# OpenRobotLab/EmbodiedScan

Measured on AMD Instinct MI355X. Metric: scans/sec (train step) mv-3ddet, 20x(480x640) RGB-D views, higher is better.
Workload: dtype bf16; 1 GPU; mv-3ddet ResNet-50(w16) + MinkResNet34 + FCAF3DHeadRotMat, 20 views 480x640, 100k points/scan, bf16 matrix cores with f32 accumulate / f32 master weights, full train step incl. H2D of the batch and AdamW; views=20, parallelism=dp1, h2d=157 MB per step as ONE copy from a pinned slab on a copy stream, double-buffered

## Files before the change

### embodiedscan_amd/csrc/rowops.hip

```cpp
#include "common.h"
#include "../../include/es_hip.h"

int ES_OPT_NORM_CHUNK = 0;
static int norm_chunk_rows(int max_rows) {
  if (ES_OPT_NORM_CHUNK > 0) return ES_OPT_NORM_CHUNK;
  return max_rows <= (1 << 17) ? 128 : (max_rows <= (1 << 18) ? 256 : 512);
}
#define FCH 16
#define FST 64

struct Segs { int n; int off[ES_MAX_SEG + 1]; };
__device__ inline int seg_of(const Segs& s, int row) {
  int g = 0;
  for (int i = 1; i < s.n; ++i) g += (row >= s.off[i]);
  return g;
}
static Segs make_segs(const int* seg_off, int nseg) {
  Segs s;
  s.n = nseg;
  for (int i = 0; i <= nseg; ++i) s.off[i] = seg_off[i];
  return s;
}
static int max_seg_rows(const Segs& s) {
  int m = 0;
// ... 258 lines not shown
                    (((((uintptr_t)x) | ((uintptr_t)y) | ((uintptr_t)res) | ((uintptr_t)weight) | ((uintptr_t)bias) |
                       ((uintptr_t)mean) | ((uintptr_t)invstd)) & 15) == 0);
  if (vec0 && norm_cb_ok(n, C, nseg) && seg_off[0] == 0 && seg_off[1] == n) {
    hipLaunchKernelGGL(k_norm_fwd_cb, dim3(C / 16), dim3(4 * NCB_TY), 0, st, x, ldx, n, C, eps, weight, bias, res, ldr, act,
                       running_mean, running_var, momentum, mean, invstd, y, ldy, (unsigned short*)y_bf16);
    ES_CHECK_LAUNCH();
    return 0;
  }
  const int NCH = norm_chunk_rows(max_seg_rows(s));
  int nchunk = es_cdiv(max_seg_rows(s), NCH);
  if (nchunk < 1) nchunk = 1;
  hipLaunchKernelGGL(k_norm_stats, dim3(nchunk, nseg), dim3(256), 0, st, x, ldx, C, s, nchunk, NCH,
                     workspace);
  hipLaunchKernelGGL(k_norm_finalize, dim3(es_cdiv(C, FCH), nseg), dim3(FCH * FST), 0, st, workspace, C, s, nchunk, NCH, eps,
                     mean, invstd, running_mean, running_var, momentum);
  const bool vec = ((C & 3) == 0) && ((ldx & 3) == 0) && ((ldy & 3) == 0) && (!res || (ldr & 3) == 0) &&
                   (((((uintptr_t)x) | ((uintptr_t)y) | ((uintptr_t)res) | ((uintptr_t)weight) | ((uintptr_t)bias) |
                      ((uintptr_t)mean) | ((uintptr_t)invstd)) & 15) == 0);
  if (vec) {
    int g = es_cdiv((long long)n * (C >> 2), 512);
    if (g > 8192) g = 8192;
    hipLaunchKernelGGL(k_norm_apply4, dim3(g < 1 ? 1 : g), dim3(256), 0, st, x, ldx, n, C, s, mean, invstd, weight, bias,
                       res, ldr, act, y, ldy, (unsigned short*)y_bf16);
  } else {
    int g = es_cdiv((long long)n * C, 256);
    if (g > 4096) g = 4096;
    hipLaunchKernelGGL(k_norm_apply, dim3(g), dim3(256), 0, st, x, ldx, n, C, s, mean, invstd, weight, bias, res,
                       ldr, act, y, ldy);
    if (y_bf16) return es_cast_rows_bf16(y, ldy, n, C, y_bf16, stream);
  }
  ES_CHECK_LAUNCH();
  return 0;
}
extern "C" size_t es_norm_workspace_floats(int n, int C, const int* seg_off, int nseg) {
  int m = 0;
  for (int i = 0; i < nseg; ++i) m = max(m, seg_off[i + 1] - seg_off[i]);
  int nchunk = es_cdiv(m, norm_chunk_rows(m));
  if (nchunk < 1) nchunk = 1;
  return (size_t)nseg * nchunk * 2 * C;
}

__global__ __launch_bounds__(256) void k_norm_bwd_stats(float* __restrict__ dy, int ldd, const float* __restrict__ y,
                                                        int ldy, const float* __restrict__ x, int ldx, int C, Segs segs,
                                                        int nchunk, int NCH, const float* __restrict__ mean,
                                                        const float* __restrict__ invstd, int act,
                                                        float* __restrict__ partial) {
  __shared__ float4 red[2][256];
  int seg = blockIdx.y, chunk = blockIdx.x;
  int r0 = segs.off[seg] + chunk * NCH, r1 = min(segs.off[seg + 1], r0 + NCH);
  float* out = partial + ((size_t)(seg * nchunk + chunk) * 2) * C;
  const bool vec = ((C & 3) == 0) && ((ldx & 3) == 0) && ((ldd & 3) == 0) && ((ldy & 3) == 0) &&
                   ((((uintptr_t)x) & 15) == 0) && ((((uintptr_t)dy) & 15) == 0) && ((((uintptr_t)y) & 15) == 0);
  if (!vec) {
    for (int c = threadIdx.x; c < C; c += blockDim.x) {
      float s = 0.f, q = 0.f, m = mean[seg * C + c], is = invstd[seg * C + c];
      for (int r = r0; r < r1; ++r) {
        float g = dy[(size_t)r * ldd + c];
        if (act) {
          float yv = y[(size_t)r * ldy + c];
          g = (act == 1) ? (yv > 0.f ? g : 0.f) : (yv > 0.f ? g : g * (yv + 1.f));
          dy[(size_t)r * ldd + c] = g;
        }
        s += g;
        q += g * ((x[(size_t)r * ldx + c] - m) * is);
      }
      out[c] = s;
      out[C + c] = q;
    }
    return;
  }
// ... 239 lines not shown
    const bool vec0 = ((C & 3) == 0) && ((ldx & 3) == 0) && ((ldd & 3) == 0) && ((ldo & 3) == 0) && ((ldy & 3) == 0) &&
                      (((((uintptr_t)x) | ((uintptr_t)dy) | ((uintptr_t)dx) | ((uintptr_t)y) | ((uintptr_t)weight) |
                         ((uintptr_t)mean) | ((uintptr_t)invstd)) & 15) == 0);
    if (vec0 && dx != dy && ES_OPT_NORM_CB_BWD && norm_cb_ok(n, C, nseg) && seg_off[0] == 0 && seg_off[1] == n) {
      hipLaunchKernelGGL(k_norm_bwd_cb, dim3(C / 16), dim3(4 * NCB_TY), 0, st, dy, ldd, y, ldy, x, ldx, n, C, mean, invstd, weight, act,
                         dweight, dbias, dx, ldo, accumulate, (unsigned short*)dx_bf16);
      ES_CHECK_LAUNCH();
      return 0;
    }
  }
  float* sums = workspace + (size_t)nseg * nchunk * 2 * C;
  hipLaunchKernelGGL(k_norm_bwd_stats, dim3(nchunk, nseg), dim3(256), 0, st, dy, ldd, y, ldy, x,
                     ldx, C, s, nchunk, NCH, mean, invstd, act, workspace);
  hipLaunchKernelGGL(k_norm_bwd_finalize, dim3(es_cdiv(C, FCH)), dim3(FCH * FST), 0, st, workspace, C, s, nchunk, NCH, sums,
                     sums + (size_t)nseg * C, dweight, dbias);
  const bool vec = ((C & 3) == 0) && ((ldx & 3) == 0) && ((ldd & 3) == 0) && ((ldo & 3) == 0) &&
                   (((((uintptr_t)x) | ((uintptr_t)dy) | ((uintptr_t)dx) | ((uintptr_t)weight) | ((uintptr_t)mean) |
                      ((uintptr_t)invstd) | ((uintptr_t)sums)) & 15) == 0) && ((((size_t)nseg * C) & 3) == 0);
  if (vec && dx != dy) {
    int g = es_cdiv((long long)n * (C >> 2), 512);
    if (g > 8192) g = 8192;
    hipLaunchKernelGGL(k_norm_bwd_apply4, dim3(g < 1 ? 1 : g), dim3(256), 0, st, dy, ldd, x, ldx, n, C, s, mean, invstd,
                       weight, sums, sums + (size_t)nseg * C, dx, ldo, accumulate, (unsigned short*)dx_bf16);
  } else {
    int g = es_cdiv((long long)n * C, 256);
    if (g > 4096) g = 4096;
    hipLaunchKernelGGL(k_norm_bwd_apply, dim3(g), dim3(256), 0, st, dy, ldd, x, ldx, n, C, s, mean, invstd, weight,
                       sums, sums + (size_t)nseg * C, dx, ldo, accumulate);
    if (dx_bf16) return es_cast_rows_bf16(dx, ldo, n, C, dx_bf16, stream);
  }
  ES_CHECK_LAUNCH();
  return 0;
}

__global__ void k_maxpool_fwd(const float* __restrict__ x, int ldx, const int* __restrict__ nbr, int n_out, int K,
                              int C, float* __restrict__ y, int* __restrict__ arg) {
  size_t tot = (size_t)n_out * C;
  for (size_t e = (size_t)blockIdx.x * blockDim.x + threadIdx.x; e < tot; e += (size_t)gridDim.x * blockDim.x) {
    int j = (int)(e / C), c = (int)(e - (size_t)j * C);
    float best = -INFINITY;
    int bi = -1;
    for (int k = 0; k < K; ++k) {
      int i = nbr[(size_t)j * K + k];
      if (i < 0) continue;
      float v = x[(size_t)i * ldx + c];
      if (bi < 0 || v > best) { best = v; bi = i; }
    }
    y[e] = best;
    arg[e] = bi;
  }
}
extern "C" int es_maxpool_fwd(const float* x, int ldx, const int* nbr, int n_out, int K, int C, float* y, int* arg,
                              void* stream) {
  if (n_out <= 0) return 0;
  int g = es_cdiv((long long)n_out * C, 256);
  if (g > 4096) g = 4096;
  hipLaunchKernelGGL(k_maxpool_fwd, dim3(g), dim3(256), 0, (hipStream_t)stream, x, ldx, nbr, n_out, K, C, y, arg);
  ES_CHECK_LAUNCH();
  return 0;
}
__global__ void k_maxpool_fwd_h(const float* __restrict__ x, int ldx, const int* __restrict__ nbr, int n_out, int K, int C,
                                unsigned short* __restrict__ y) {
  size_t tot = (size_t)n_out * C;
  for (size_t e = (size_t)blockIdx.x * blockDim.x + threadIdx.x; e < tot; e += (size_t)gridDim.x * blockDim.x) {
    int j = (int)(e / C), c = (int)(e - (size_t)j * C);
    float best = -INFINITY;
// ... 552 lines not shown
```

### embodiedscan_amd/csrc/spconv.hip

```cpp
#include "common.h"
#include "../../include/es_hip.h"

typedef float f32x4 __attribute__((ext_vector_type(4)));

static int ES_OPT_PINGPONG = 1;
static int ES_OPT_WGRAD_HUGE = 1;
static int ES_OPT_ROWGEMM = 1;
static int ES_OPT_WG_BIG_TARGET = 2048;
static int ES_OPT_WG_BIG_ROWS = 512;
static int ES_OPT_WG_SMALL_TARGET = 1024;
static int ES_OPT_WG_CAP_MB = 256;
static int ES_OPT_FWD_SPLIT_WGS = 384;
static int ES_OPT_DMA = 2;
static int ES_OPT_DMA_MIN_CIN = 768;
static int ES_OPT_WGRAD_TR = 1;
static int ES_OPT_ROWGEMM2 = 1;
static int ES_OPT_SPLIT_FOLD = 0;
static int ES_OPT_RG128_MIN_CIN = 0;
static int ES_OPT_NARROW_SLICES = 768;
static int ES_OPT_LIN_SMALL = 256;
static int ES_OPT_EXPAND = 65536;
static int ES_OPT_EXPAND_WGS = 1024;
static int ES_OPT_RG320 = 1;
static int ES_OPT_NARROW = 1;
static int ES_OPT_WSHARE = 0;
static int ES_OPT_RG128_MIN_WGS = 0;
extern int ES_OPT_NORM_CB_ROWS;
extern int ES_OPT_NORM_CB_BWD;
extern int ES_OPT_ELECT_SAFE;
extern int ES_OPT_NORM_CHUNK;
extern "C" int es_set_option(int key, int value) {
  if (key == 1) { ES_OPT_PINGPONG = value; return 0; }
  if (key == 2) { ES_OPT_WGRAD_HUGE = value; return 0; }
  if (key == 3) { ES_OPT_ROWGEMM = value; return 0; }
  if (key == 4) { ES_OPT_WG_BIG_TARGET = value; return 0; }
  if (key == 5) { ES_OPT_WG_BIG_ROWS = value; return 0; }
  if (key == 6) { ES_OPT_WG_SMALL_TARGET = value; return 0; }
  if (key == 7) { ES_OPT_WG_CAP_MB = value; return 0; }
  if (key == 8) { ES_OPT_FWD_SPLIT_WGS = value; return 0; }
  if (key == 9) { ES_OPT_NORM_CHUNK = value; return 0; }
  if (key == 10) { ES_OPT_DMA = value; return 0; }
  if (key == 11) { ES_OPT_DMA_MIN_CIN = value; return 0; }
  if (key == 12) { ES_OPT_RG128_MIN_CIN = value; return 0; }
  if (key == 13) { ES_OPT_ROWGEMM2 = value; return 0; }
  if (key == 14) { ES_OPT_WGRAD_TR = value; return 0; }
  if (key == 15) { ES_OPT_NORM_CB_ROWS = value; return 0; }
  if (key == 16) { ES_OPT_SPLIT_FOLD = value; return 0; }
  if (key == 17) { ES_OPT_NORM_CB_BWD = value; return 0; }
  if (key == 18) { ES_OPT_ELECT_SAFE = value; return 0; }
  if (key == 19) { ES_OPT_RG128_MIN_WGS = value; return 0; }
  if (key == 20) { ES_OPT_WSHARE = value; return 0; }
  if (key == 21) { ES_OPT_NARROW = value; return 0; }
  if (key == 22) { ES_OPT_NARROW_SLICES = value; return 0; }
  if (key == 23) { ES_OPT_RG320 = value; return 0; }
  if (key == 24) { ES_OPT_LIN_SMALL = value; return 0; }
  if (key == 25) { ES_OPT_EXPAND = value; return 0; }
  if (key == 26) { ES_OPT_EXPAND_WGS = value; return 0; }
  return -2;
}


#define BM 128
#define BN 64
#define BK 16
#define LDB (BN + 16)
#define MAXK 27

__device__ inline int a_swz(int row_k) { return (((row_k >> 2) & 3) << 3) ^ ((row_k & 1) << 4); }

template <bool TRANS_W>
__global__ __launch_bounds__(256) void k_spconv(const float* __restrict__ X, int ldx, const float* __restrict__ W,
                                                const int* __restrict__ nbr, int n_out, int n_in, int K, int Cin,
                                                int Cout, const float* __restrict__ bias, float* __restrict__ Y,
                                                int ldy, int accumulate) {
  __shared__ float As[BK * BM];
  __shared__ float Bs[BK * LDB];
  __shared__ int nbrS[BM * MAXK];
  __shared__ int tapAny[32];

  const int t = threadIdx.x, lane = t & 63, wv = t >> 6;
  const int row0 = blockIdx.x * BM, n0 = blockIdx.y * BN;
  const bool vecA = ((ldx & 3) == 0) && ((((uintptr_t)X) & 15) == 0);
  const bool vecB = TRANS_W ? (((Cin & 3) == 0) && ((((uintptr_t)W) & 15) == 0))
                            : (((Cout & 3) == 0) && ((((uintptr_t)W) & 15) == 0));

  if (t < 32) tapAny[t] = 0;
  __syncthreads();
  for (int e = t; e < BM * K; e += 256) {
    int r = e / K, k = e - r * K;
    int j = row0 + r, v = -1;
// ... 2674 lines not shown
```

### embodiedscan_amd/engine.py

```python
import os

import torch
from . import hip
from .hip import P, call, iarr


def _stream():
    return hip.stream()


_NEW_VARS = None


class Var:
    __slots__ = ('d', 'g', 'rg', 'dh', 'gh', 'gate', 'gated', 'fresh')

    def __init__(self, d, rg=True):
        self.d, self.g, self.rg = d, None, rg
        self.dh = self.gh = None
        if _NEW_VARS is not None:
            _NEW_VARS.append(self)
        self.fresh = False
        self.gate = None
        self.gated = False
# ... 407 lines not shown
def _cast_rows(t):
    n, C = t.shape
    h = torch.empty((n, C), dtype=torch.bfloat16, device=t.device)
    call('es_cast_rows_bf16', P(t), t.stride(0), n, C, P(h), _stream())
    return h


GEN_FUSED = [os.environ.get('ES_GEN_FUSED', '1') != '0']


def _split_ws(n_out, K, cin, cout, like):
    if K <= 1 or n_out <= 0:
        return None, 0
    nf = int(hip.raw('es_spconv_split_workspace_floats')(n_out, K, cin, cout))
    if nf == 0:
        return None, 0
    return ticket_ws(nf, like, tag='split')


def _fwd_bf16(X, x_is_bf16, ldx, Wp, nbr, n_out, n_in, K, cin, cout, bias_p, Y, ldy, acc, like):
    ws, nf = _split_ws(n_out, K, cin, cout, like)
    if ws is not None:
        call('es_spconv_fwd_bf16_ws', X, x_is_bf16, ldx, Wp, nbr, n_out, n_in, K, cin, cout, bias_p, Y, ldy, acc, P(ws), nf, _stream())
        return 'es_spconv_fwd_bf16_ws'
    call('es_spconv_fwd_bf16', X, x_is_bf16, ldx, Wp, nbr, n_out, n_in, K, cin, cout, bias_p, Y, ldy, acc, _stream())
    return 'es_spconv_fwd_bf16'


def _use_shadow(n_rows, C, K, cin, cout):
    return K > 1 and hip.raw('es_spconv_bf16_is_fast')(n_rows, C, K, cin, cout) == 1


HALO = [os.environ.get('ES_HALO', '1') != '0']
if os.environ.get('ES_HALO_MIN_WGS') is not None:
    hip.raw('es_halo_set_option')(30, int(os.environ['ES_HALO_MIN_WGS']))


def _halo_ok(nbr, n_out, n_in, ldx, K, cin, cout):
    return (HALO[0] and K == 27 and nbr is not None
            and hip.raw('es_spconv_halo_supported')(n_out, n_in, ldx, K, cin, cout) == 1)


def halo_plan(nbr):
    plan = getattr(nbr, '_halo', None)
    if plan is None:
        n_out, K = nbr.shape
        rows = int(hip.raw('es_halo_plan_rows')(n_out))
        loc = torch.empty((rows, K), dtype=torch.int16, device=nbr.device)
        hrows = torch.empty((rows // 256, 256 * K), dtype=torch.int32, device=nbr.device)
        hcnt = torch.empty((rows // 256,), dtype=torch.int32, device=nbr.device)
        call('es_halo_plan', P(nbr), n_out, K, P(loc), P(hrows), P(hcnt), _stream())
        plan = nbr._halo = (loc, hrows, hcnt)
        if hip.PROFILE is not None:
            hip.PAIRS[loc.data_ptr()] = (nbr >= 0).sum()
    return plan


def _halo_launch(Xh, ldx, Wp, nbr, n_out, n_in, K, cin, cout, bias_p, Y, ldy, acc):
    fwd = getattr(nbr, '_mirror_of', None)
    loc, hrows, hcnt = halo_plan(fwd if fwd is not None else nbr)
    return hip.try_call('es_spconv_halo_bf16', Xh, ldx, Wp, P(loc), P(hrows), P(hcnt), n_out, n_in, K, cin, cout, bias_p, Y, ldy, acc,
                        int(fwd is not None), _stream())


def empty(shape, like, dtype=torch.float32):
    return torch.empty(shape, dtype=dtype, device=like.device)
# ... 347 lines not shown
            x.shadow()
            sw = _wgrad_stream(y.g, x.d, gh, x.dh)
            _required(_dense_wgrad(P(x.dh), cin, P(gh), cout, dense, 1, cin, cout, P(w.g), _first_write(P(w.g)), sw, gh))
        if x.rg:
            g, acc = _grad_target(x, x.d)
            _required(_dense_launch(P(gh), cout, P(w.bf16()[0]), dense, 4, cin, cout, P(g), _ld(g), acc, gh))
        if DEBUG_CONV is not None:
            B, X, Y, Z = dense[:4]
            gv = y.g.view(B, X, 2, Y, 2, Z, 2, cout)
            recs = [dict(x=x.d, w=ParamSlice(w, k), nbr=None, n_out=n, gy=gv[:, :, k >> 2, :, (k >> 1) & 1, :, k & 1].reshape(n, cout).clone(),
                         bf=True, gate=None, need_dx=bool(x.rg), before=rec_before, bias=None, bias_from=0, group=id(y), group_size=8)
                    for k in range(8)]
            if x.rg:
                recs[-1]['after'] = x.g.clone()
            DEBUG_CONV.extend(recs)
    TAPE.add(bwd)
    return y


def norm(x, weight, bias, seg_off, eps, act=0, res=None, running=None, momentum=0.1):
    n, C = x.d.shape
    nseg = len(seg_off) - 1
    so = iarr(seg_off)
    ws_n = hip.raw('es_norm_workspace_floats')(n, C, so, nseg) + 2 * nseg * C
    ws = empty((ws_n,), x.d)
    mean, invstd = empty((nseg, C), x.d), empty((nseg, C), x.d)
    y = Var(empty((n, C), x.d))
    rm, rv = (running if running is not None else (None, None))
    fuse = PRECISION[0] == 'bf16' and C >= 16 and C % 8 == 0
    private, x.fresh = bool(x.fresh), False
    if fuse:
        y.dh = empty((n, C), x.d, dtype=torch.bfloat16)
    run0 = (rm.clone(), rv.clone()) if (DEBUG_FWD is not None and rm is not None) else (None, None)
    call('es_norm_fwd', P(x.d), _ld(x.d), n, C, so, nseg, float(eps), P(weight.d), P(bias.d),
         P(res.d) if res is not None else 0, _ld(res.d) if res is not None else 0, act, P(rm), P(rv), float(momentum),
         P(mean), P(invstd), P(ws), P(y.d), C, P(y.dh) if fuse else 0, _stream())
    if DEBUG_FWD is not None:
        fwd_record('norm', 'es_norm_fwd', x=x.d, w=weight.d, b=bias.d, seg_off=list(seg_off), eps=float(eps), act=act,
                   res=res.d if res is not None else None, rm0=run0[0], rv0=run0[1], rm1=rm, rv1=rv, momentum=float(momentum),
                   mean=mean, invstd=invstd, y=y.d, yh=y.dh if fuse else None)

    def bwd():
        if y.g is None:
            return
        s = _stream()
        if DEBUG_GRADS is not None:
            DEBUG_GRADS[id(y)] = y.g.clone()
        ws2 = empty((ws_n,), x.d)
        g, acc = _grad_target(x, x.d)
        gh = empty((n, C), x.d, dtype=torch.bfloat16) if (fuse and private and _ld(g) == C) else None
        call('es_norm_bwd', P(y.g), _ld(y.g), P(y.d), C, P(x.d), _ld(x.d), n, C, so, nseg, P(mean), P(invstd),
             P(weight.d), act, P(weight.g), P(bias.g), P(ws2), P(g), _ld(g), acc, P(gh), s)
        x.gh = gh
        if DEBUG_GRADS is not None:
            DEBUG_GRADS[('norm', id(y))] = dict(dx=g.clone(), dz=y.g.clone(), mean=mean.clone(), invstd=invstd.clone(),
                                                x=x.d.clone(), yd=y.d.clone(), acc=acc, n=n, C=C, act=act)
        if res is not None and res.rg:
            if res.g is None:
                res.g = y.g
            else:
                call('es_axpy2d', P(res.g), _ld(res.g), P(y.g), _ld(y.g), n, C, 1.0, 1, s)
    TAPE.add(bwd)
    return y


def affine_act(x, scale, shift, act=1, res=None, need_dx=True):
    n, C = x.d.shape
    y = Var(empty((n, C), x.d))
    call('es_affine_act_fwd', P(x.d), P(scale), P(shift), P(res.d) if res is not None else 0, n, C, act, P(y.d),
         _stream())
    if DEBUG_FWD is not None:
        fwd_record('affine_act', 'es_affine_act_fwd', x=x.d, scale=scale, shift=shift, res=res.d if res is not None else None,
                   act=act, y=y.d)

    def bwd():
        if y.g is None:
            return
        gx = accx = gr = accr = 0
        if need_dx and x.rg:
            t, accx = _grad_target(x, x.d)
            gx = P(t)
        if res is not None and res.rg:
            t, accr = _grad_target(res, res.d)
            gr = P(t)
        if gx or gr:
            call('es_affine_act_bwd', P(y.g), P(y.d), P(scale), n, C, act, gx, accx, gr, accr, _stream())
    TAPE.add(bwd)
    return y

# ... 241 lines not shown
```

### embodiedscan_amd/hip.py

```python
import ctypes
import os
import re

_HERE = os.path.dirname(os.path.abspath(__file__))
LIB_PATH = os.path.join(_HERE, 'libes_hip.so')
HEADER_PATH = os.path.join(os.path.dirname(_HERE), 'include', 'es_hip.h')

_CT = {'int': ctypes.c_int, 'float': ctypes.c_float, 'double': ctypes.c_double, 'size_t': ctypes.c_size_t}


def parse_header(path=HEADER_PATH):
    src = open(path).read()
    src = re.sub(r'/\*.*?\*/', ' ', src, flags=re.S)
    out = {}
    for m in re.finditer(r'\b(int|size_t)\s+(es_\w+)\s*\(([^)]*)\)\s*;', src):
        ret, name, args = m.group(1), m.group(2), m.group(3)
        at, an = [], []
        for a in args.split(','):
            a = a.strip()
            if not a or a == 'void':
                continue
            an.append(re.findall(r'(\w+)\s*$', a)[0])
            if '*' in a:
                at.append(ctypes.c_void_p)
            else:
                toks = [t for t in a.split() if t != 'const']
                at.append(_CT[toks[0]])
        out[name] = (_CT[ret], at, an)
    return out


PROTOS = parse_header()
CONSTS = {k: int(v) for k, v in re.findall(r'#define\s+(ES_\w+)\s+(\d+)', open(HEADER_PATH).read())}

if not os.path.exists(LIB_PATH):
    raise ImportError(f'{LIB_PATH} is missing: build it with `make -C embodiedscan_amd/csrc` '
                      '(or __graft_entry__.build()); there is no CPU fallback for the HIP path')
_lib = ctypes.CDLL(LIB_PATH)
_fn = {}
for _name, (_ret, _at, _an) in PROTOS.items():
    _f = getattr(_lib, _name)
    _f.restype, _f.argtypes = _ret, _at
    _fn[_name] = _f


if os.environ.get('ES_PINGPONG') is not None:
    _fn['es_set_option'](1, int(os.environ['ES_PINGPONG']))
if os.environ.get('ES_WGRAD_HUGE') is not None:
    _fn['es_set_option'](2, int(os.environ['ES_WGRAD_HUGE']))
if os.environ.get('ES_ROWGEMM') is not None:
    _fn['es_set_option'](3, int(os.environ['ES_ROWGEMM']))
for _key, _env in ((4, 'ES_WG_BIG_TARGET'), (5, 'ES_WG_BIG_ROWS'), (6, 'ES_WG_SMALL_TARGET'), (7, 'ES_WG_CAP_MB'), (8, 'ES_FWD_SPLIT_WGS'),
                  (10, 'ES_DMA'), (11, 'ES_DMA_MIN_CIN'), (12, 'ES_RG128_MIN_CIN'), (14, 'ES_WGRAD_TR'), (15, 'ES_NORM_CB_ROWS'),
                  (16, 'ES_SPLIT_FOLD'), (19, 'ES_RG128_MIN_WGS'), (20, 'ES_WSHARE'), (21, 'ES_NARROW'), (23, 'ES_RG320'), (24, 'ES_LIN_SMALL'), (25, 'ES_EXPAND'), (26, 'ES_EXPAND_WGS')):
    if os.environ.get(_env) is not None:
        _fn['es_set_option'](_key, int(os.environ[_env]))


class HipError(RuntimeError):
    pass


PROFILE = None
PAIRS = {}


def register_map(nbr):
    if PROFILE is not None and nbr is not None:
        PAIRS[nbr.data_ptr()] = (nbr >= 0).sum()
    return nbr


_EXT_STREAMS = {}


def _stream_of(handle):
    import torch
    st = _EXT_STREAMS.get(handle)
    if st is None:
        st = _EXT_STREAMS[handle] = torch.cuda.ExternalStream(handle) if handle else torch.cuda.default_stream()
    return st


def _launch(name, args):
    prof = PROFILE
    if prof is not None and name in prof['names']:
        e0, e1 = prof['event'](), prof['event']()
# ... 66 lines not shown
```

### include/es_hip.h

```cpp
#ifndef ES_HIP_H
#define ES_HIP_H
#include <stddef.h>
#include <stdint.h>
#ifdef __cplusplus
extern "C" {
#endif

#define ES_MAX_SEG 32

#define ES_MAX_BATCH 512
int es_voxel_keys(const float* points, int n, int ld, int batch, float voxel_size, int64_t* keys, void* stream);
int es_unique_first(const int64_t* keys, int n, int64_t* tkeys, int* tvals, int cap, int* scratch,
                    int64_t* out_keys, int* out_src, int* count_host, void* stream);
size_t es_sort_scratch_bytes(int n);
int es_morton_sort(const int64_t* keys, const int* src, int n, void* scratch, size_t scratch_bytes, int64_t* out_keys,
                   int* out_src, void* stream);
int es_sort_u64(const int64_t* keys, const int* src, int n, void* scratch, size_t scratch_bytes, int64_t* out_keys, int* out_src,
                void* stream);
int es_draw_keys(const float* depth, int V, int HW, size_t seed, float* values, int64_t* keys, void* stream);
int es_draw_keys_index(int n, size_t seed, int stream_id, float* values, int64_t* keys, void* stream);
int es_draw_unpack(const int64_t* keys, int n, const int* in_view, const int* in_pix, int* out_view, int* out_pix, void* stream);
int es_build_table(const int64_t* keys, int n, int64_t* tkeys, int* tvals, int cap, void* stream);
int es_stride_keys(const int64_t* in_keys, int n, int out_ts, int64_t* out_keys, void* stream);
int es_keys_to_coords(const int64_t* keys, int n, int* coords , void* stream);
// ... 26 lines not shown
int es_gen_transpose_fwd_bf16(const float* X, int ldx, const void* Wt_bf16, int n, int Cin, int Cout, float* Y, void* stream);
int es_gen_transpose_dgrad_bf16(const float* dY, const void* Wn_bf16, int n, int Cin, int Cout, float* dX, int ldx,
                                int accumulate, void* stream);
int es_set_option(int key, int value);
int es_spconv_fwd_bf16_affine(const void* X, int ldx, const void* W_bf16, const int* nbr, int n_out, int n_in, int K,
                              int Cin, int Cout, const float* scale, const float* shift, const float* res, int ldr,
                              int act, float* Y, int ldy, void* stream);
int es_spconv_fwd_bf16_io(const void* X, int x_half, int ldx, const void* W_bf16, const int* nbr, int n_out, int n_in, int K,
                          int Cin, int Cout, const float* scale, const float* shift, const void* res, int res_half, int ldr,
                          int act, void* Y, int y_half, int ldy, void* stream);
int es_cast_rows_bf16(const float* x, int ldx, int n, int C, void* h , void* stream);
int es_cast_weight_bf16(const float* w, int K, int A, int B, void* natural, void* transposed, void* stream);
int es_cast_weights_table(const void* table_dev, int n_entries, int total_tiles, void* stream);
int es_spconv_wgrad(const float* X, int ldx, const float* dY, int ldy, const int* nbr, int n_out, int n_in, int K,
                    int Cin, int Cout, float* dW, int accumulate, float* ws, size_t ws_floats, void* stream);
int es_spconv_wgrad_bf16(const float* X, int ldx, const float* dY, int ldy, const int* nbr, int n_out, int n_in, int K,
                         int Cin, int Cout, float* dW, int accumulate, float* ws, size_t ws_floats, void* stream);
int es_spconv_wgrad_bf16_src(const void* X, int x_half, int ldx, const void* dY, int dy_half, int ldy, const int* nbr,
                             int n_out, int n_in, int K, int Cin, int Cout, float* dW, int accumulate, float* ws,
                             size_t ws_floats, void* stream);
size_t es_spconv_wgrad_workspace_floats(int bf16, const void* X, int x_half, int ldx, const void* dY, int dy_half, int ldy,
                                        int n_out, int n_in, int K, int Cin, int Cout);
int es_image_map(int n_img, int H, int W, int Ho, int Wo, int KH, int KW, int stride, int pad, int* nbr, void* stream);

size_t es_norm_workspace_floats(int n, int C, const int* seg_off_host, int nseg);
int es_norm_fwd(const float* x, int ldx, int n, int C, const int* seg_off_host, int nseg, float eps,
                const float* weight, const float* bias, const float* res, int ldr, int act, float* running_mean,
                float* running_var, float momentum, float* mean, float* invstd, float* workspace, float* y, int ldy,
                void* y_bf16, void* stream);
int es_norm_bwd(float* dy, int ldd, const float* y, int ldy, const float* x, int ldx, int n, int C,
                const int* seg_off_host, int nseg, const float* mean, const float* invstd, const float* weight,
                int act, float* dweight, float* dbias, float* workspace, float* dx, int ldo, int accumulate,
                void* dx_bf16, void* stream);
int es_maxpool_fwd(const float* x, int ldx, const int* nbr, int n_out, int K, int C, float* y, int* arg, void* stream);
int es_maxpool_fwd_h(const float* x, int ldx, const int* nbr, int n_out, int K, int C, void* y_bf16, void* stream);
int es_maxpool_bwd(const float* dy, const int* arg, int n_out, int C, float* dx, int ldo, void* stream);
int es_row_move(float* dst, int ldd, const float* src, int lds, const int* idx, int n, int C, int mode, void* stream);
int es_axpy2d(float* dst, int ldd, const float* src, int lds, int n, int C, float alpha, int op, void* stream);
int es_interp_scores(const float* score, const int* idx, const float* w, int n, float* out, void* stream);
size_t es_colsum_workspace_floats(int n, int C);
int es_colsum(const float* g, int ld, int n, int C, float* dst, int accumulate, float* workspace, size_t workspace_floats, void* stream);
int es_topk_mask(const float* values, const int* seg_off_host, int nseg, int k, int* mask, void* stream);
size_t es_topk_mask_workspace_ints(int nseg);
int es_topk_mask_ws(const float* values, const int* seg_off_host, int nseg, int k, int* mask, int* workspace, size_t workspace_ints,
                    void* stream);
int es_row_max(const float* x, int ldx, int n, int C, float* out, void* stream);
int es_bn_fold(const float* w, const float* b, const float* rm, const float* rv, int C, float eps, float* scale,
               float* shift, void* stream);
int es_affine_act_fwd(const float* x, const float* scale, const float* shift, const float* res, size_t n, int C,
                      int act, float* y, void* stream);
int es_affine_act_bwd(const float* dy, const float* y, const float* scale, size_t n, int C, int act, float* dx,
                      int acc_x, float* dres, int acc_r, void* stream);
int es_affine_act_bwd_yh(const float* dy, const void* y_bf16, const float* scale, size_t n, int C, int act, float* dx,
                         int acc_x, float* dres, int acc_r, void* stream);

#define ES_FUSE_NOPS 0
#define ES_FUSE_OPS 1
#define ES_FUSE_ROTINV 9
#define ES_FUSE_ISCALE 18
#define ES_FUSE_NTRANS 19
#define ES_FUSE_SFX 22
#define ES_FUSE_SFY 23
#define ES_FUSE_CROPX 24
#define ES_FUSE_CROPY 25
#define ES_FUSE_FLIP 26
#define ES_FUSE_ORIW 27
// ... 185 lines not shown
```

Baseline: 176.5 scans/s.

## Add wide-norm path merging partial-stat reduction into the apply kernel

New measurement: 176.9 scans/s, median of 2. About the same (+0.2%).

```diff
diff --git a/embodiedscan_amd/csrc/rowops.hip b/embodiedscan_amd/csrc/rowops.hip
--- a/embodiedscan_amd/csrc/rowops.hip
+++ b/embodiedscan_amd/csrc/rowops.hip
@@ -314,10 +314,204 @@
   ES_CHECK_LAUNCH();
   return 0;
 }
+int ES_OPT_NORM_WIDE = 1;
+int ES_OPT_NORM_WIDE_ROWS = 32;
+int ES_OPT_NORM_WIDE_BWD_ROWS = 32;
+int ES_OPT_NORM_MERGE_MAX = 64;
+#define NM_CW 64
+#define NM_ROWS 32
+static int norm_merge_max() { return ES_OPT_NORM_MERGE_MAX < 1 ? 1 : (ES_OPT_NORM_MERGE_MAX > FST ? FST : ES_OPT_NORM_MERGE_MAX); }
+static int norm_wide_chunk(int n, int base) {
+  int r = base < 1 ? 1 : base;
+  while (es_cdiv(n, r) > norm_merge_max()) r *= 2;
+  return r;
+}
+__device__ inline void nm_stage(const float* __restrict__ partial, int C, int c0, int cw, int used, float* rec) {
+  float4 v[8];
+  const int tot = used * 2 * (NM_CW / 4);
+#pragma unroll
+  for (int i = 0; i < 8; ++i) {
+    const int idx = threadIdx.x + 256 * i, rh = idx >> 4, c4 = (idx & 15) * 4;
+    v[i] = make_float4(0, 0, 0, 0);
+    if (idx < tot && c4 < cw) v[i] = *(const float4*)(partial + (size_t)rh * C + c0 + c4);
+  }
+#pragma unroll
+  for (int i = 0; i < 8; ++i) {
+    const int idx = threadIdx.x + 256 * i;
+    if (idx < tot) *(float4*)(rec + (size_t)idx * 4) = v[i];
+  }
+}
+template <typename TV>
+__device__ inline double nm_seqsum(const TV* p, int stride, int used) {
+  double tot = 0;
+  for (int s0 = 0; s0 < used; s0 += 8) {
+    double v[8];
+#pragma unroll
+    for (int u = 0; u < 8; ++u) {
+      const int ch = s0 + u;
+      const TV xv = p[(size_t)min(ch, used - 1) * stride];
+      v[u] = ch < used ? (double)xv : 0.0;
+    }
+#pragma unroll
+    for (int u = 0; u < 8; ++u) tot += v[u];
+  }
+  return tot;
+}
+__global__ __launch_bounds__(256) void k_norm_apply_merge(const float* __restrict__ x, int ldx, int n, int C,
+                                                          const float* __restrict__ partial, int used, int NCH, float eps,
+                                                          const float* __restrict__ w, const float* __restrict__ b,
+                                                          const float* __restrict__ res, int ldr, int act, float* running_mean,
+                                                          float* running_var, float momentum, float* __restrict__ mean,
+                                                          float* __restrict__ invstd, float* __restrict__ y, int ldy,
+                                                          unsigned short* __restrict__ yh) {
+  extern __shared__ float nm_rec[];
+  __shared__ double nm_m[NM_CW];
+  __shared__ __attribute__((aligned(16))) float nm_out[2][NM_CW];
+  const int t = threadIdx.x, tx = t & 15, ty = t >> 4;
+  const int c0 = blockIdx.y * NM_CW, cw = min(NM_CW, C - c0), c = c0 + tx * 4;
+  const bool col = tx * 4 < cw;
+  const int r0 = blockIdx.x * NM_ROWS + ty, r1 = r0 + 16;
+  const bool v0 = col && r0 < n, v1 = col && r1 < n;
+  float4 x0 = make_float4(0, 0, 0, 0), x1 = x0, q0 = x0, q1 = x0;
+  if (v0) x0 = *(const float4*)(x + (size_t)r0 * ldx + c);
+  if (v1) x1 = *(const float4*)(x + (size_t)r1 * ldx + c);
+  if (res && v0) q0 = *(const float4*)(res + (size_t)r0 * ldr + c);
+  if (res && v1) q1 = *(const float4*)(res + (size_t)r1 * ldr + c);
+  nm_stage(partial, C, c0, cw, used, nm_rec);
+  __syncthreads();
+  if (t < NM_CW) nm_m[t] = nm_seqsum(nm_rec + t, 2 * NM_CW, used) / n;
+  __syncthreads();
+  {
+    const int cl = t & 63, j = t >> 6;
+    const double m = nm_m[cl];
+    const bool pow2 = (NCH & (NCH - 1)) == 0;
+    const double inv_nch = 1.0 / NCH;
+    double term[FST / 4];
+#pragma unroll
+    for (int i = 0; i < FST / 4; ++i) {
+      const int ch = j + 4 * i;
+      term[i] = 0;
+      if (ch < used) {
+        const int nc = min(NCH, n - ch * NCH);
+        const double sc = (double)nm_rec[(ch * 2) * NM_CW + cl], qc = (double)nm_rec[(ch * 2 + 1) * NM_CW + cl];
+        double d;
+        if (pow2 && nc == NCH) d = sc * inv_nch - m;
+        else d = sc / nc - m;
+        term[i] = qc + nc * d * d;
+      }
+    }
+    __syncthreads();
+    double* terms = (double*)nm_rec;
+#pragma unroll
+    for (int i = 0; i < FST / 4; ++i) {
+      const int ch = j + 4 * i;
+      if (ch < used) terms[ch * NM_CW + cl] = term[i];
+    }
+  }
+  __syncthreads();
+  if (t < NM_CW) {
+    const double m = nm_m[t], m2 = nm_seqsum((const double*)nm_rec + t, NM_CW, used);
+    const double var = m2 / n;
+    const float mf = (float)m, isf = (float)(1.0 / sqrt(var + (double)eps));
+    nm_out[0][t] = mf;
+    nm_out[1][t] = isf;
+    if (blockIdx.x == 0 && t < cw) {
+      mean[c0 + t] = mf;
+      invstd[c0 + t] = isf;
+      if (running_mean && n > 1) {
+        running_mean[c0 + t] = (1.f - momentum) * running_mean[c0 + t] + momentum * (float)m;
+        running_var[c0 + t] = (1.f - momentum) * running_var[c0 + t] + momentum * (float)(var * n / (n - 1));
+      }
+    }
+  }
+  __syncthreads();
+  if (!v0) return;
+  const float4 m = *(const float4*)(nm_out[0] + tx * 4), is = *(const float4*)(nm_out[1] + tx * 4);
+  const float4 ww = *(const float4*)(w + c), bb = *(const float4*)(b + c);
+#define NM_ONE(xv, qv, r)                                                                                      \
+  {                                                                                                            \
+    float z0 = (xv.x - m.x) * is.x * ww.x + bb.x, z1 = (xv.y - m.y) * is.y * ww.y + bb.y;                      \
+    float z2 = (xv.z - m.z) * is.z * ww.z + bb.z, z3 = (xv.w - m.w) * is.w * ww.w + bb.w;                      \
+    if (res) { z0 += qv.x; z1 += qv.y; z2 += qv.z; z3 += qv.w; }                                               \
+    z0 = act_fwd(z0, act); z1 = act_fwd(z1, act); z2 = act_fwd(z2, act); z3 = act_fwd(z3, act);               \
+    *(float4*)(y + (size_t)(r) * ldy + c) = make_float4(z0, z1, z2, z3);                                       \
+    if (yh) *(uint2*)(yh + (size_t)(r) * C + c) = make_uint2(es_pack_bf16(z0, z1), es_pack_bf16(z2, z3));      \
+  }
+  NM_ONE(x0, q0, r0)
+  if (v1) NM_ONE(x1, q1, r1)
+#undef NM_ONE
+}
+static bool norm_wide_fwd_ok(const float* x, int ldx, int n, int C, const int* seg_off, int nseg, const float* weight,
+                             const float* bias, const float* res, int ldr, const float* mean, const float* invstd, const float* y,
+                             int ldy) {
+  return ES_OPT_NORM_WIDE && nseg == 1 && seg_off[0] == 0 && seg_off[1] == n && ((C & 3) == 0) && ((ldx & 3) == 0) &&
+         ((ldy & 3) == 0) && (!res || (ldr & 3) == 0) &&
+         (((((uintptr_t)x) | ((uintptr_t)y) | ((uintptr_t)res) | ((uintptr_t)weight) | ((uintptr_t)bias) | ((uintptr_t)mean) |
+            ((uintptr_t)invstd)) & 15) == 0);
+}
+extern "C" int es_norm_stats_tiles(const float* x, int ldx, int n, int C, int tile_rows, float* partial, void* stream) {
+  if (n <= 0) return 0;
+  if (tile_rows < 1) return -1;
+  Segs s;
+  s.n = 1; s.off[0] = 0; s.off[1] = n;
+  const int nchunk = es_cdiv(n, tile_rows);
+  hipLaunchKernelGGL(k_norm_stats, dim3(nchunk, 1), dim3(256), 0, (hipStream_t)stream, x, ldx, C, s, nchunk, tile_rows, partial);
+  ES_CHECK_LAUNCH();
+  return 0;
+}
+extern "C" int es_norm_fwd_partials(const float* x, int ldx, int n, int C, const int* seg_off, int nseg, float eps,
+                                    const float* weight, const float* bias, const float* res, int ldr, int act,
+                                    float* running_mean, float* running_var, float momentum, float* mean, float* invstd,
+                                    float* workspace, float* y, int ldy, void* y_bf16, const float* partial, int n_tiles,
+                                    int tile_rows, void* stream) {
+  hipStream_t st = (hipStream_t)stream;
+  (void)workspace;
+  if (n <= 0) return 0;
+  if (!norm_wide_fwd_ok(x, ldx, n, C, seg_off, nseg, weight, bias, res, ldr, mean, invstd, y, ldy)) return -4;
+  if (!partial || tile_rows < 1 || n_tiles != es_cdiv(n, tile_rows)) return -1;
+  if (n_tiles > norm_merge_max() || (((uintptr_t)partial) & 15)) {
+    Segs s = make_segs(seg_off, 1);
+    hipLaunchKernelGGL(k_norm_finalize, dim3(es_cdiv(C, FCH), 1), dim3(FCH * FST), 0, st, partial, C, s, n_tiles, tile_rows, eps, mean,
+                       invstd, running_mean, running_var, momentum);
+    int g = es_cdiv((long long)n * (C >> 2), 512);
+    if (g > 8192) g = 8192;
+    hipLaunchKernelGGL(k_norm_apply4, dim3(g < 1 ? 1 : g), dim3(256), 0, st, x, ldx, n, C, s, mean, invstd, weight, bias, res, ldr,
+                       act, y, ldy, (unsigned short*)y_bf16);
+  } else {
+    hipLaunchKernelGGL(k_norm_apply_merge, dim3(es_cdiv(n, NM_ROWS), es_cdiv(C, NM_CW)), dim3(256),
+                       (size_t)n_tiles * 2 * NM_CW * sizeof(float), st, x, ldx, n, C, partial, n_tiles, tile_rows, eps, weight, bias,
+                       res, ldr, act, running_mean, running_var, momentum, mean, invstd, y, ldy, (unsigned short*)y_bf16);
+  }
+  ES_CHECK_LAUNCH();
+  return 0;
+}
+extern "C" int es_norm_fwd_wide(const float* x, int ldx, int n, int C, const int* seg_off, int nseg, float eps,
+                                const float* weight, const float* bias, const float* res, int ldr, int act,
+                                float* running_mean, float* running_var, float momentum, float* mean, float* invstd,
+                                float* workspace, float* y, int ldy, void* y_bf16, void* stream) {
+  if (n <= 0) return 0;
+  const int rows = norm_wide_chunk(n, ES_OPT_NORM_WIDE_ROWS);
+  if (!norm_cb_ok(n, C, nseg) || (((uintptr_t)workspace) & 15) ||
+      !norm_wide_fwd_ok(x, ldx, n, C, seg_off, nseg, weight, bias, res, ldr, mean, invstd, y, ldy))
+    return -4;
+  int rc = es_norm_stats_tiles(x, ldx, n, C, rows, workspace, stream);
+  if (rc) return rc;
+  return es_norm_fwd_partials(x, ldx, n, C, seg_off, nseg, eps, weight, bias, res, ldr, act, running_mean, running_var, momentum,
+                              mean, invstd, workspace, y, ldy, y_bf16, workspace, es_cdiv(n, rows), rows, stream);
+}
+extern "C" int es_norm_wide_rows(int n, int C, int backward) {
+  if (!ES_OPT_NORM_WIDE || n < 1 || (C & 3) || !norm_cb_ok(n, C, 1)) return 0;
+  return norm_wide_chunk(n, backward ? ES_OPT_NORM_WIDE_BWD_ROWS : ES_OPT_NORM_WIDE_ROWS);
+}
 extern "C" size_t es_norm_workspace_floats(int n, int C, const int* seg_off, int nseg) {
   int m = 0;
   for (int i = 0; i < nseg; ++i) m = max(m, seg_off[i + 1] - seg_off[i]);
   int nchunk = es_cdiv(m, norm_chunk_rows(m));
+  if (nseg == 1) {
+    const int wr[2] = {ES_OPT_NORM_WIDE_ROWS, ES_OPT_NORM_WIDE_BWD_ROWS};
+    for (int i = 0; i < 2; ++i)
+      if (norm_cb_ok(m, C, 1)) nchunk = max(nchunk, es_cdiv(m, norm_wide_chunk(m, wr[i])));
+  }
   if (nchunk < 1) nchunk = 1;
   return (size_t)nseg * nchunk * 2 * C;
 }
@@ -623,6 +817,74 @@
   ES_CHECK_LAUNCH();
   return 0;
 }
+__global__ __launch_bounds__(256) void k_norm_bwd_apply_merge(const float* __restrict__ dz, int ldd, const float* __restrict__ x,
+                                                              int ldx, int n, int C, const float* __restrict__ partial, int used,
+                                                              const float* __restrict__ mean, const float* __restrict__ invstd,
+                                                              const float* __restrict__ w, float* dweight, float* dbias,
+                                                              float* __restrict__ dx, int ldo, int accumulate,
+                                                              unsigned short* __restrict__ dxh) {
+  extern __shared__ float nm_rec[];
+  const int t = threadIdx.x, tx = t & 15, ty = t >> 4;
+  const int c0 = blockIdx.y * NM_CW, cw = min(NM_CW, C - c0), c = c0 + tx * 4;
+  const bool col = tx * 4 < cw;
+  const int r0 = blockIdx.x * NM_ROWS + ty, r1 = r0 + 16;
+  const bool v0 = col && r0 < n, v1 = col && r1 < n;
+  float4 x0 = make_float4(0, 0, 0, 0), x1 = x0, g0 = x0, g1 = x0, o0 = x0, o1 = x0;
+  if (v0) { x0 = *(const float4*)(x + (size_t)r0 * ldx + c); g0 = *(const float4*)(dz + (size_t)r0 * ldd + c); }
+  if (v1) { x1 = *(const float4*)(x + (size_t)r1 * ldx + c); g1 = *(const float4*)(dz + (size_t)r1 * ldd + c); }
+  if (accumulate && v0) o0 = *(const float4*)(dx + (size_t)r0 * ldo + c);
+  if (accumulate && v1) o1 = *(const float4*)(dx + (size_t)r1 * ldo + c);
+  nm_stage(partial, C, c0, cw, used, nm_rec);
+  __syncthreads();
+  float tot = 0.f;
+  const int h = t >> 6, cl = t & 63;
+  if (h < 2) tot = (float)nm_seqsum(nm_rec + h * NM_CW + cl, 2 * NM_CW, used);
+  __syncthreads();
+  if (h < 2) {
+    nm_rec[h * NM_CW + cl] = tot;
+    float* dpar = h ? dweight : dbias;
+    if (blockIdx.x == 0 && cl < cw && dpar) dpar[c0 + cl] += tot;
+  }
+  __syncthreads();
+  if (!v0) return;
+  const float4 sd = *(const float4*)(nm_rec + tx * 4), sq = *(const float4*)(nm_rec + NM_CW + tx * 4);
+  const float4 m = *(const float4*)(mean + c), is = *(const float4*)(invstd + c), ww = *(const float4*)(w + c);
+  const float inv_n = 1.f / (float)n;
+#define NBM_ELT(xe, ge, oe, me, ie, we, se, qe) \
+  { float xh = ((xe) - (me)) * (ie); float gg = (we) * (ie) * ((ge) - (se) * inv_n - xh * (qe) * inv_n); oe = accumulate ? ((oe) + gg) : gg; }
+#define NBM_ONE(xv, gv, ov, r)                                                                                 \
+  {                                                                                                            \
+    NBM_ELT(xv.x, gv.x, ov.x, m.x, is.x, ww.x, sd.x, sq.x) NBM_ELT(xv.y, gv.y, ov.y, m.y, is.y, ww.y, sd.y, sq.y) \
+    NBM_ELT(xv.z, gv.z, ov.z, m.z, is.z, ww.z, sd.z, sq.z) NBM_ELT(xv.w, gv.w, ov.w, m.w, is.w, ww.w, sd.w, sq.w) \
+    *(float4*)(dx + (size_t)(r) * ldo + c) = ov;                                                               \
+    if (dxh) *(uint2*)(dxh + (size_t)(r) * C + c) = make_uint2(es_pack_bf16(ov.x, ov.y), es_pack_bf16(ov.z, ov.w)); \
+  }
+  NBM_ONE(x0, g0, o0, r0)
+  if (v1) NBM_ONE(x1, g1, o1, r1)
+#undef NBM_ONE
+#undef NBM_ELT
+}
+extern "C" int es_norm_bwd_wide(float* dy, int ldd, const float* y, int ldy, const float* x, int ldx, int n, int C,
+                                const int* seg_off, int nseg, const float* mean, const float* invstd, const float* weight,
+                                int act, float* dweight, float* dbias, float* workspace, float* dx, int ldo, int accumulate,
+                                void* dx_bf16, void* stream) {
+  hipStream_t st = (hipStream_t)stream;
+  if (n <= 0) return 0;
+  const int rows = norm_wide_chunk(n, ES_OPT_NORM_WIDE_BWD_ROWS);
+  const bool vec = ((C & 3) == 0) && ((ldx & 3) == 0) && ((ldd & 3) == 0) && ((ldo & 3) == 0) && ((ldy & 3) == 0) &&
+                   (((((uintptr_t)x) | ((uintptr_t)dy) | ((uintptr_t)dx) | ((uintptr_t)y) | ((uintptr_t)weight) | ((uintptr_t)mean) |
+                      ((uintptr_t)invstd) | ((uintptr_t)workspace)) & 15) == 0);
+  if (!ES_OPT_NORM_WIDE || nseg != 1 || seg_off[0] != 0 || seg_off[1] != n || !vec || dx == dy || !norm_cb_ok(n, C, 1)) return -4;
+  Segs s = make_segs(seg_off, 1);
+  const int nchunk = es_cdiv(n, rows);
+  hipLaunchKernelGGL(k_norm_bwd_stats, dim3(nchunk, 1), dim3(256), 0, st, dy, ldd, y, ldy, x, ldx, C, s, nchunk, rows, mean, invstd,
+                     act, workspace);
+  hipLaunchKernelGGL(k_norm_bwd_apply_merge, dim3(es_cdiv(n, NM_ROWS), es_cdiv(C, NM_CW)), dim3(256),
+                     (size_t)nchunk * 2 * NM_CW * sizeof(float), st, dy, ldd, x, ldx, n, C, workspace, nchunk, mean, invstd, weight,
+                     dweight, dbias, dx, ldo, accumulate, (unsigned short*)dx_bf16);
+  ES_CHECK_LAUNCH();
+  return 0;
+}
 
 __global__ void k_maxpool_fwd(const float* __restrict__ x, int ldx, const int* __restrict__ nbr, int n_out, int K,
                               int C, float* __restrict__ y, int* __restrict__ arg) {
diff --git a/embodiedscan_amd/csrc/spconv.hip b/embodiedscan_amd/csrc/spconv.hip
--- a/embodiedscan_amd/csrc/spconv.hip
+++ b/embodiedscan_amd/csrc/spconv.hip
@@ -29,6 +29,10 @@
 extern int ES_OPT_NORM_CB_BWD;
 extern int ES_OPT_ELECT_SAFE;
 extern int ES_OPT_NORM_CHUNK;
+extern int ES_OPT_NORM_WIDE;
+extern int ES_OPT_NORM_WIDE_ROWS;
+extern int ES_OPT_NORM_WIDE_BWD_ROWS;
+extern int ES_OPT_NORM_MERGE_MAX;
 extern "C" int es_set_option(int key, int value) {
   if (key == 1) { ES_OPT_PINGPONG = value; return 0; }
   if (key == 2) { ES_OPT_WGRAD_HUGE = value; return 0; }
@@ -56,6 +60,10 @@
   if (key == 24) { ES_OPT_LIN_SMALL = value; return 0; }
   if (key == 25) { ES_OPT_EXPAND = value; return 0; }
   if (key == 26) { ES_OPT_EXPAND_WGS = value; return 0; }
+  if (key == 27) { ES_OPT_NORM_WIDE = value; return 0; }
+  if (key == 28) { ES_OPT_NORM_WIDE_ROWS = value; return 0; }
+  if (key == 29) { ES_OPT_NORM_WIDE_BWD_ROWS = value; return 0; }
+  if (key == 32) { ES_OPT_NORM_MERGE_MAX = value; return 0; }
   return -2;
 }
 
diff --git a/embodiedscan_amd/engine.py b/embodiedscan_amd/engine.py
--- a/embodiedscan_amd/engine.py
+++ b/embodiedscan_amd/engine.py
@@ -463,6 +463,8 @@
 
 
 HALO = [os.environ.get('ES_HALO', '1') != '0']
+NORM_FUSED = [os.environ.get('ES_NORM_FUSED', '1') != '0']
+NORM_WIDE_FWD = [os.environ.get('ES_NORM_WIDE_FWD', '0') == '1']
 if os.environ.get('ES_HALO_MIN_WGS') is not None:
     hip.raw('es_halo_set_option')(30, int(os.environ['ES_HALO_MIN_WGS']))
 
@@ -876,13 +878,16 @@
     if fuse:
         y.dh = empty((n, C), x.d, dtype=torch.bfloat16)
     run0 = (rm.clone(), rv.clone()) if (DEBUG_FWD is not None and rm is not None) else (None, None)
-    call('es_norm_fwd', P(x.d), _ld(x.d), n, C, so, nseg, float(eps), P(weight.d), P(bias.d),
-         P(res.d) if res is not None else 0, _ld(res.d) if res is not None else 0, act, P(rm), P(rv), float(momentum),
-         P(mean), P(invstd), P(ws), P(y.d), C, P(y.dh) if fuse else 0, _stream())
+    fargs = (P(x.d), _ld(x.d), n, C, so, nseg, float(eps), P(weight.d), P(bias.d),
+             P(res.d) if res is not None else 0, _ld(res.d) if res is not None else 0, act, P(rm), P(rv), float(momentum),
+             P(mean), P(invstd), P(ws), P(y.d), C, P(y.dh) if fuse else 0, _stream())
+    wide = NORM_FUSED[0] and NORM_WIDE_FWD[0] and nseg == 1 and hip.try_call('es_norm_fwd_wide', *fargs)
+    if not wide:
+        call('es_norm_fwd', *fargs)
     if DEBUG_FWD is not None:
         fwd_record('norm', 'es_norm_fwd', x=x.d, w=weight.d, b=bias.d, seg_off=list(seg_off), eps=float(eps), act=act,
                    res=res.d if res is not None else None, rm0=run0[0], rv0=run0[1], rm1=rm, rv1=rv, momentum=float(momentum),
-                   mean=mean, invstd=invstd, y=y.d, yh=y.dh if fuse else None)
+                   mean=mean, invstd=invstd, y=y.d, yh=y.dh if fuse else None, path='wide' if wide else None)
 
     def bwd():
         if y.g is None:
@@ -893,12 +898,16 @@
         ws2 = empty((ws_n,), x.d)
         g, acc = _grad_target(x, x.d)
         gh = empty((n, C), x.d, dtype=torch.bfloat16) if (fuse and private and _ld(g) == C) else None
-        call('es_norm_bwd', P(y.g), _ld(y.g), P(y.d), C, P(x.d), _ld(x.d), n, C, so, nseg, P(mean), P(invstd),
-             P(weight.d), act, P(weight.g), P(bias.g), P(ws2), P(g), _ld(g), acc, P(gh), s)
+        bargs = (P(y.g), _ld(y.g), P(y.d), C, P(x.d), _ld(x.d), n, C, so, nseg, P(mean), P(invstd),
+                 P(weight.d), act, P(weight.g), P(bias.g), P(ws2), P(g), _ld(g), acc, P(gh), s)
+        wide_b = NORM_FUSED[0] and nseg == 1 and hip.try_call('es_norm_bwd_wide', *bargs)
+        if not wide_b:
+            call('es_norm_bwd', *bargs)
         x.gh = gh
         if DEBUG_GRADS is not None:
             DEBUG_GRADS[('norm', id(y))] = dict(dx=g.clone(), dz=y.g.clone(), mean=mean.clone(), invstd=invstd.clone(),
-                                                x=x.d.clone(), yd=y.d.clone(), acc=acc, n=n, C=C, act=act)
+                                                x=x.d.clone(), yd=y.d.clone(), acc=acc, n=n, C=C, act=act,
+                                                path='wide' if wide_b else None)
         if res is not None and res.rg:
             if res.g is None:
                 res.g = y.g
diff --git a/embodiedscan_amd/hip.py b/embodiedscan_amd/hip.py
--- a/embodiedscan_amd/hip.py
+++ b/embodiedscan_amd/hip.py
@@ -52,7 +52,8 @@
     _fn['es_set_option'](3, int(os.environ['ES_ROWGEMM']))
 for _key, _env in ((4, 'ES_WG_BIG_TARGET'), (5, 'ES_WG_BIG_ROWS'), (6, 'ES_WG_SMALL_TARGET'), (7, 'ES_WG_CAP_MB'), (8, 'ES_FWD_SPLIT_WGS'),
                   (10, 'ES_DMA'), (11, 'ES_DMA_MIN_CIN'), (12, 'ES_RG128_MIN_CIN'), (14, 'ES_WGRAD_TR'), (15, 'ES_NORM_CB_ROWS'),
-                  (16, 'ES_SPLIT_FOLD'), (19, 'ES_RG128_MIN_WGS'), (20, 'ES_WSHARE'), (21, 'ES_NARROW'), (23, 'ES_RG320'), (24, 'ES_LIN_SMALL'), (25, 'ES_EXPAND'), (26, 'ES_EXPAND_WGS')):
+                  (16, 'ES_SPLIT_FOLD'), (19, 'ES_RG128_MIN_WGS'), (20, 'ES_WSHARE'), (21, 'ES_NARROW'), (23, 'ES_RG320'), (24, 'ES_LIN_SMALL'), (25, 'ES_EXPAND'), (26, 'ES_EXPAND_WGS'),
+                  (27, 'ES_NORM_FUSED'), (28, 'ES_NORM_WIDE_ROWS'), (29, 'ES_NORM_WIDE_BWD_ROWS'), (32, 'ES_NORM_MERGE_MAX')):
     if os.environ.get(_env) is not None:
         _fn['es_set_option'](_key, int(os.environ[_env]))
 
diff --git a/include/es_hip.h b/include/es_hip.h
--- a/include/es_hip.h
+++ b/include/es_hip.h
@@ -82,6 +82,20 @@
                 const int* seg_off_host, int nseg, const float* mean, const float* invstd, const float* weight,
                 int act, float* dweight, float* dbias, float* workspace, float* dx, int ldo, int accumulate,
                 void* dx_bf16, void* stream);
+int es_norm_fwd_wide(const float* x, int ldx, int n, int C, const int* seg_off_host, int nseg, float eps,
+                     const float* weight, const float* bias, const float* res, int ldr, int act, float* running_mean,
+                     float* running_var, float momentum, float* mean, float* invstd, float* workspace, float* y, int ldy,
+                     void* y_bf16, void* stream);
+int es_norm_bwd_wide(float* dy, int ldd, const float* y, int ldy, const float* x, int ldx, int n, int C,
+                     const int* seg_off_host, int nseg, const float* mean, const float* invstd, const float* weight,
+                     int act, float* dweight, float* dbias, float* workspace, float* dx, int ldo, int accumulate,
+                     void* dx_bf16, void* stream);
+int es_norm_wide_rows(int n, int C, int backward);
+int es_norm_stats_tiles(const float* x, int ldx, int n, int C, int tile_rows, float* partial, void* stream);
+int es_norm_fwd_partials(const float* x, int ldx, int n, int C, const int* seg_off_host, int nseg, float eps,
+                         const float* weight, const float* bias, const float* res, int ldr, int act, float* running_mean,
+                         float* running_var, float momentum, float* mean, float* invstd, float* workspace, float* y, int ldy,
+                         void* y_bf16, const float* partial, int n_tiles, int tile_rows, void* stream);
 int es_maxpool_fwd(const float* x, int ldx, const int* nbr, int n_out, int K, int C, float* y, int* arg, void* stream);
 int es_maxpool_fwd_h(const float* x, int ldx, const int* nbr, int n_out, int K, int C, void* y_bf16, void* stream);
 int es_maxpool_bwd(const float* dy, const int* arg, int n_out, int C, float* dx, int ldo, void* stream);
```
